# hchautran/SplatFormer

Hardware: AMD Instinct MI355X
Metric: refined renders/sec (100k GS, 800x800) at 1/2/4/8 MI355X; PSNR vs ref (higher is better)
Workload: dtype fp32; 1 GPU; B: 100000 Gaussians SH1, full PTv3 (ptv3_base) + heads, 9 views 800x800, forward; parallelism=scene-dp1, attention=non-flash (K=128, ptv3_base.gin:27)

## Files before the change

### include/sfx.h

```cpp
#ifndef SFX_H_
#define SFX_H_

#include <stddef.h>
#include <stdint.h>

#ifdef __cplusplus
extern "C" {
#endif

#define SFX_OK 0
#define SFX_ERR_INVALID -1
#define SFX_ERR_HIP -2
#define SFX_ERR_WORKSPACE -3

int sfx_abi_version(void);
const char* sfx_last_error(void);

size_t sfx_scan_workspace_bytes(long long n);
long long sfx_lookback_timeouts(void* stream);
int sfx_lookback_release(void* stream);
int sfx_scan_i32(long long n, const int32_t* in, int32_t* out, int inclusive, void* ws, size_t ws_bytes,
                 int32_t* total, void* stream);
int sfx_scan_i64(long long n, const int64_t* in, int64_t* out, int inclusive, void* ws, size_t ws_bytes,
                 int64_t* total, void* stream);
// ... 17 lines not shown
                    const float* v_conic, const float* v_compensation, float* v_mean, float* v_scale,
                    float* v_quat, float* v_cov2d, float* v_cov3d, void* stream);

int sfx_render_prep_project(int n, int num_bases, const float* means, long long ld_means, const float* log_scales,
                            long long ld_scales, const float* quats_raw, long long ld_quats, const float* opac_logit,
                            long long ld_opac, const float* features_dc, long long ld_dc, const float* features_rest,
                            long long ld_rest, const float* camera_to_world, float fx, float fy, float cx,
                            float cy, int img_h, int img_w, int block_width, float* viewmat_out, float* rgbs,
                            float* opacities, float* xys, float* depths, int* radii, float* conics,
                            int* num_tiles_hit, void* stream);

int sfx_isect_emit(int n, const float* xys, const float* depths, const int* radii, const int* cum_tiles_hit,
                   int tiles_x, int tiles_y, int block_width, int64_t* isect_ids, int32_t* gaussian_ids,
                   void* stream);
int sfx_tile_bins(int num_isect, const int64_t* isect_ids_sorted, int num_tiles, int* tile_bins, void* stream);

int sfx_rasterize_fwd(int tiles_x, int tiles_y, int block_width, int img_h, int img_w, const int32_t* gids_sorted,
                      const int* tile_bins, const float* xys, const float* conics, const float* colors,
                      const float* opacity, const float* background, float* final_Ts, int* final_idx,
                      float* out_img, float* out_alpha, void* stream);
int sfx_rasterize_bwd(int tiles_x, int tiles_y, int block_width, int img_h, int img_w, const int32_t* gids_sorted,
                      const int* tile_bins, const float* xys, const float* conics, const float* colors,
                      const float* opacity, const float* background, const float* final_Ts, const int* final_idx,
                      const float* v_out, const float* v_out_alpha, float* v_xy, float* v_xy_abs, float* v_conic,
                      float* v_rgb, float* v_opacity, void* stream);

int sfx_pack_raster_records(int n, const float* xys, const float* conics, const float* colors, const float* opacity,
                            float* records, void* stream);
int sfx_rasterize_fwd_views_packed(int views, int tiles_x, int tiles_y, int block_width, int img_h, int img_w,
                                   const int32_t* gids_sorted, const int* tile_bins, const float* records,
                                   const float* background, int clamp_max1, float* final_Ts, int* final_idx,
                                   float* out_img, float* out_alpha, void* stream);

int sfx_linear(int M, int N, int K, const float* A, long long lda, const int* gather_idx, int num_segments,
               const float* W, long long ldw, const float* bias, const float* scale, const float* shift, int act,
               int act_ncols, const float* R, long long ldr, const int* residual_idx, float* Y, long long ldy,
               float* Ypre, long long ldypre, int groups, long long group_stride_A, long long group_stride_W,
               long long group_stride_bias, long long group_stride_Y, const int* out_row_idx, const float* rowscale,
               int pre_before_act, const unsigned long long* a_amax, unsigned a_tag,
               const unsigned long long* w_amax, unsigned w_tag, unsigned long long* y_amax, unsigned y_tag,
               const float* w_split, const float* w_inv, void* stream);

int sfx_weight_split(int rows, int cols, const float* w, long long ld, float* w_split, float* w_inv, void* stream);

int sfx_amax_f32(int rows, int cols, const float* x, long long ld, unsigned long long* slot, unsigned tag,
                 void* stream);
int sfx_ln_amax_bound(int C, const float* gamma, const float* beta, unsigned long long* slot, unsigned tag,
                      void* stream);

int sfx_gemm_force_config(int cfg, int stream_k);

int sfx_gemm_force_epilogue(int cls);
int sfx_gemm_last_epilogue(void);

int sfx_set_precision(int mode);
int sfx_get_precision(void);

int sfx_linear_bwd_data(int M, int N, int K, const float* dY, long long ldy, const float* Wt, long long ldwt,
                        const float* rowscale, int dact, int dact_ncols, const float* dact_pre, long long ld_pre,
                        float* dX, long long lddx, int accumulate, const float* wt_split, const float* wt_inv,
                        void* stream);
int sfx_linear_wgrad(int M, int N, int K, const float* dY, long long ldy, const float* X, long long ldx, float* dW,
                     long long ldw, float* db, void* stream);
int sfx_linear_wgrad_rs(int M, int N, int K, const float* dY, long long ldy, const float* X, long long ldx,
                        const float* rowscale, float* scaled, float* dW, long long ldw, float* db, void* stream);
int sfx_subm_conv_wgrad(int n, int cin, int cout, const float* dy, long long ldy, const float* x, long long ldx,
                        const int* nbr, const int* pair_in, const int* pair_out, const int* pair_off_host, float* dw,
                        long long ldw, float* db, void* stream);
int sfx_profile_marker(int tag, void* stream);

int sfx_transpose(int rows, int cols, const float* src, long long lds, float* dst, long long ldd, void* stream);
int sfx_subm_conv_bwd_data(int n, int cin, int cout, const float* dy, long long ldy, const int* nbr,
                           const float* weight_t, const int* pair_in, const int* pair_out, const int* pair_off_host,
                           int* centre_ws, float* dx, long long lddx, const float* wt_split, const float* wt_inv,
                           void* stream);
int sfx_window_attention_bwd(int num_windows, int window, int heads, int head_dim, int channels, const float* qkv,
                             const int* order, const int* win, float scale, const float* attn_out, const float* dout,
                             float* dqkv, float* stats, void* stream);
int sfx_window_attention_varlen_bwd(int num_windows, int max_window, int heads, int head_dim, int channels,
                                    const float* qkv, const int* order, const int* win3, float scale,
                                    const float* dout, float* dqkv, float* stats, void* stream);
int sfx_layernorm_bwd(int M, int C, const float* X, long long ldx, const float* gamma, const float* dY,
                      long long ldgy, const float* dR, long long ldr, float eps, float* dX, long long lddx,
                      void* stream);
size_t sfx_layernorm_wgrad_workspace_bytes(int M, int C);
int sfx_layernorm_wgrad(int M, int C, const float* X, long long ldx, const float* dY, long long ldgy, float eps,
                        void* ws, size_t ws_bytes, float* dgamma, float* dbeta, int accumulate, void* stream);
int sfx_cpe_ln_bwd(int M, int C, const float* U, const float* X1, const float* gamma_cpe, const float* gamma1,
                   const float* dX2, const float* dH, float eps, float* dX1, float* dU, void* stream);
size_t sfx_colsum2_workspace_bytes(int M, int C);
int sfx_bn_stats(int M, int C, const float* X, long long ldx, void* ws, size_t ws_bytes, double* sums, void* stream);
int sfx_bn_finalize(int C, double count, const double* sums, const float* gamma, const float* beta, float eps,
                    float momentum, float* running_mean, float* running_var, float* mean_out, float* rstd_out,
                    float* scale_out, float* shift_out, void* stream);
int sfx_affine_act(int M, int C, const float* X, long long ldx, const float* scale, const float* shift, int act,
                   const float* R, long long ldr, const int* ridx, float* Y, long long ldy, void* stream);
int sfx_bn_act_bwd_reduce(int M, int C, const float* X, long long ldx, const float* mean, const float* rstd,
                          const float* gamma, const float* beta, int act, const float* dY, long long ldgy, void* ws,
                          size_t ws_bytes, double* sums, void* stream);
int sfx_bn_act_bwd_apply(int M, int C, const float* X, long long ldx, const float* mean, const float* rstd,
                         const float* gamma, const float* beta, int act, const float* dY, long long ldgy,
                         const double* sums, double count, float* dX, long long lddx, int accumulate, void* stream);
int sfx_segment_max_arg(int m, int C, const int* idx_ptr, const int* sorted_idx, const float* X, float* Y, int* arg,
                        void* stream);
int sfx_segment_max_bwd(int m, int C, const float* dY, const int* arg, float* dX, void* stream);
int sfx_segment_sum(int m, int C, const int* idx_ptr, const int* sorted_idx, const float* X, long long ldx, float* Y,
// ... 211 lines not shown
```

### splatformer_amd/build_lib.py

```python
from __future__ import annotations

import concurrent.futures as cf
import glob
import os
import re
import subprocess
import sys

HERE = os.path.dirname(os.path.abspath(__file__))
CSRC = os.path.join(HERE, "csrc")
ROOT = os.path.dirname(HERE)
BUILD = os.path.join(ROOT, "build", "sfx")
LIB = os.path.join(HERE, "libsfx.so")
ARCH = os.environ.get("SFX_OFFLOAD_ARCH", "gfx950")
HIPCC = os.environ.get("HIPCC", "/opt/rocm/bin/hipcc")

CFLAGS = [
    f"--offload-arch={ARCH}",
    "-O3",
    "-fPIC",
    "-std=c++17",
    "-ffp-contract=fast-honor-pragmas",
    "-munsafe-fp-atomics",
    "-Wno-unused-result",
    f"-I{CSRC}",
    f"-I{os.path.join(ROOT, 'include')}",
]


_INC = re.compile(r'^\s*#\s*include\s*"([^"]+)"', re.M)


def _deps_mtime(path: str, seen=None) -> float:
    seen = set() if seen is None else seen
    if path in seen or not os.path.exists(path):
        return 0.0
    seen.add(path)
    t = os.path.getmtime(path)
    for inc in _INC.findall(open(path, errors="ignore").read()):
        for d in (os.path.dirname(path), CSRC, os.path.join(ROOT, "include")):
            cand = os.path.join(d, inc)
            if os.path.exists(cand):
                t = max(t, _deps_mtime(cand, seen))
                break
    return t


def _flags_stamp() -> float:
    stamp = os.path.join(BUILD, "flags.txt")
    want = " ".join([HIPCC, *CFLAGS])
    have = open(stamp).read() if os.path.exists(stamp) else None
    if have != want:
        with open(stamp, "w") as f:
            f.write(want)
    return os.path.getmtime(stamp)


def _compile(src: str, flags_mtime: float) -> str:
    obj = os.path.join(BUILD, os.path.basename(src).replace(".hip", ".o"))
    if os.path.exists(obj) and os.path.getmtime(obj) >= max(_deps_mtime(src), flags_mtime):
        return obj
    cmd = [HIPCC, *CFLAGS, "-c", src, "-o", obj]
    r = subprocess.run(cmd, capture_output=True, text=True)
    if r.returncode != 0:
        raise RuntimeError(f"hipcc failed for {src}:\n{r.stderr}")
    return obj


def build(verbose: bool = False, jobs: int | None = None) -> str:
    os.makedirs(BUILD, exist_ok=True)
    srcs = sorted(glob.glob(os.path.join(CSRC, "*.hip")))
    hm = _flags_stamp()
    jobs = jobs or min(8, len(srcs))
    with cf.ThreadPoolExecutor(jobs) as ex:
        objs = list(ex.map(lambda s: _compile(s, hm), srcs))
    newest = max(os.path.getmtime(o) for o in objs)
    if not os.path.exists(LIB) or os.path.getmtime(LIB) < newest:
        cmd = [HIPCC, f"--offload-arch={ARCH}", "-shared", "-fPIC", "-o", LIB, *objs]
        r = subprocess.run(cmd, capture_output=True, text=True)
        if r.returncode != 0:
            raise RuntimeError(f"link failed:\n{r.stderr}")
    if verbose:
        print(f"built {LIB}")
    return LIB


if __name__ == "__main__":
    build(verbose=True)
    sys.exit(0)
```

### splatformer_amd/csrc/gemm.hip

```cpp
#include <climits>
#include <cstdlib>
#include <cstring>
#include <type_traits>

#include "gemm_common.h"


namespace {

using namespace sfxg;

inline bool aligned16(const void* p) { return (reinterpret_cast<uintptr_t>(p) & 15) == 0; }

inline bool fits(long long rows, long long ld) { return rows * ld * 4 + 64 < (long long)OOB; }

struct TileCfg {
  int bm, bn, nw;
  float eff;
};
constexpr TileCfg kCfgs[] = {{128, 128, 4, 1.0f}, {128, 96, 4, 0.95f}, {128, 64, 4, 0.8f}, {64, 128, 4, 0.95f},
                             {64, 64, 4, 0.8f},   {256, 128, 8, 1.05f}, {128, 256, 8, 1.05f}};
constexpr int kNumCfgs = sizeof(kCfgs) / sizeof(kCfgs[0]);

thread_local int g_prec = 0;
// ... 204 lines not shown
    for (const TunedLaunch& t : kTuned) {
      if (t.N == a.N && t.K == a.K && 5ll * a.M >= 4ll * t.M && 4ll * a.M <= 5ll * t.M &&
          !((kCfgs[t.cfg].nw == 8) && !split)) {
        a.sk = (t.sk && sk_ok && kCfgs[t.cfg].bm >= 128) ? 1 : 0;
        tiles_m_of(a, kCfgs[t.cfg].bm);
        return t.cfg;
      }
    }
  }
  int best = 0;
  bool best_sk = false;
  double best_cost = 1e300;
  for (int c = 0; c < kNumCfgs; ++c) {
    if (force >= 0 && c != force) continue;
    if (kCfgs[c].nw == 8 && !split) continue;
    const int per_cu = kCfgs[c].nw == 4 ? kPerCu4 : kPerCu8;
    const long long slots = (long long)per_cu * num_cus() / groups;
    const double area = (double)kCfgs[c].bm * kCfgs[c].bn / kCfgs[c].eff * per_cu / 2;
    const long long tiles = (long long)tiles_m_of(a, kCfgs[c].bm) * sfx::ceil_div(a.N, kCfgs[c].bn) * groups;
    const long long rounds = (tiles + slots - 1) / slots;
    double cost = (double)rounds * (nk + 1) * area;
    bool sk = false;
    if (sk_ok && kCfgs[c].bm >= 128) {
      const double sk_cost = ((double)((tiles * nk + slots - 1) / slots) + sk_overhead) * area;
      if (sk_cost < cost || forced_sk == 1) {
        cost = sk_cost;
        sk = true;
      }
    }
    if (cost < best_cost) {
      best_cost = cost;
      best = c;
      best_sk = sk;
    }
  }
  a.sk = best_sk ? 1 : 0;
  tiles_m_of(a, kCfgs[best].bm);
  return best;
}

int forced_epi = -2;
int last_epi = -1;
int pick_epi(const GemmArgs& a, bool vec) {
  if (forced_epi == -2) {
    const char* e = getenv("SFX_GEMM_EPI");
    forced_epi = (e && *e && atoi(e) == 0) ? 0 : -1;
  }
  if (forced_epi == 0 || !vec || a.split != 2 || a.sk) return EPI_GENERAL;
  if (a.pair_mode) return a.pair_store ? EPI_PAIR_STORE : EPI_GENERAL;
  if (a.gidx || a.out_rows || a.ridx || a.Ypre || a.rowscale || a.dact) return EPI_GENERAL;
  return a.act == ACT_NONE ? EPI_LIN : (a.act == ACT_GELU ? EPI_LIN_GELU : EPI_GENERAL);
}

template <int MODE>
void dispatch_mode(GemmArgs a, int groups, bool vec, hipStream_t st) {
  const int cfg = pick_cfg(a, groups, vec);
  a.epi = last_epi = pick_epi(a, vec);
  const bool w8 = kCfgs[cfg].nw == 8;
  switch (MODE) {
    case MODE_DENSE: (w8 ? launch_m0_w8 : launch_m0_w4)(cfg, a, groups, vec, st); break;
    case MODE_GATHER1: (w8 ? launch_m1_w8 : launch_m1_w4)(cfg, a, groups, vec, st); break;
    default: (w8 ? launch_m3_w8 : launch_m3_w4)(cfg, a, groups, vec, st); break;
  }
}

void dispatch(const GemmArgs& a0, int groups, bool vec, hipStream_t st) {
  GemmArgs a = a0;
  static const int dbg = getenv("SFX_GEMM_DEBUG") ? atoi(getenv("SFX_GEMM_DEBUG")) : 0;
  a.dbg = dbg;
  a.split = vec ? split_mode(a.K) : 0;
  if (a.split == 2 && !a.Wsp) a.split = 3;
  if (a.split == 2 && g_prec == 1) a.split = 1;
  last_epi = EPI_GENERAL;
  if (a.pair_mode)
    dispatch_mode<MODE_PAIR>(a, groups, vec, st);
  else if (!a.gidx)
    dispatch_mode<MODE_DENSE>(a, groups, vec, st);
  else if (a.S == 1)
    dispatch_mode<MODE_GATHER1>(a, groups, vec, st);
  else
    launch_m2_w4(3, a, groups, vec, st);
}

__global__ void __launch_bounds__(256) weight_split_kernel(int rows, int cols, const float* __restrict__ src,
                                                           long long ld, float* __restrict__ dst,
                                                           float* __restrict__ inv) {
  const int row = (int)blockIdx.x * 4 + (int)(threadIdx.x >> 6);
  const int lane = threadIdx.x & 63;
  if (row >= rows) return;
  const float* s = src + (long long)row * ld;
  float m = 0.f;
  for (int c = lane * 4; c < cols; c += 256) {
    const float4 v = *reinterpret_cast<const float4*>(s + c);
    m = fmaxf(m, fmaxf(fmaxf(fabsf(v.x), fabsf(v.y)), fmaxf(fabsf(v.z), fabsf(v.w))));
  }
  m = sfx::wave_max(m);
  int e = 0;
  if (m > 0.f && m <= 3.4028235e38f) e = row_exp(m) + 2;
  const float sc = ldexpf(1.f, e);
  uint2* d = reinterpret_cast<uint2*>(dst + (long long)row * cols);
  for (int c = lane * 4; c < cols; c += 256) {
    uint2 t[2];
    split2h(*reinterpret_cast<const float4*>(s + c), sc, t);
    d[c / 2] = t[0];
    d[c / 2 + 1] = t[1];
  }
  if (lane == 0) inv[row] = ldexpf(1.f, -e);
}

constexpr int WG_TILE = 64;

__global__ void __launch_bounds__(THREADS) wgrad_kernel(int M, int N, int K, const float* __restrict__ dY,
                                                        long long ldy, const float* __restrict__ X, long long ldx,
                                                        float* __restrict__ dW, long long ldw, int chunk,
                                                        float* __restrict__ db) {
  __shared__ __attribute__((aligned(16))) float sA[WG_TILE * LDS_STRIDE];
  __shared__ __attribute__((aligned(16))) float sB[WG_TILE * LDS_STRIDE];
  const int tiles_k = (K + WG_TILE - 1) / WG_TILE;
  const int n0 = (blockIdx.x / tiles_k) * WG_TILE, k0 = (blockIdx.x % tiles_k) * WG_TILE;
  const int m_begin = blockIdx.y * chunk;
  const int m_end = min(M, m_begin + chunk);
  const int tid = threadIdx.x, lane = tid & 63, wid = tid >> 6;
// ... 234 lines not shown
                                                            float* __restrict__ out) {
  const long long i = (long long)blockIdx.x * 256 + threadIdx.x;
  if (i >= (long long)M * n4) return;
  const int m = (int)(i / n4), c = (int)(i % n4) * 4;
  const float s = rowscale[m];
  const float4 v = *reinterpret_cast<const float4*>(dY + (long long)m * ldy + c);
  *reinterpret_cast<float4*>(out + i * 4) = make_float4(v.x * s, v.y * s, v.z * s, v.w * s);
}

__global__ void __launch_bounds__(256) transpose_kernel(int rows, int cols, const float* __restrict__ src,
                                                        long long lds, float* __restrict__ dst, long long ldd) {
  __shared__ float t[32][33];
  const int r0 = blockIdx.y * 32, c0 = blockIdx.x * 32;
  const int tx = threadIdx.x & 31, ty = threadIdx.x >> 5;
  for (int i = ty; i < 32; i += 8) {
    const int r = r0 + i, c = c0 + tx;
    t[i][tx] = (r < rows && c < cols) ? src[(long long)r * lds + c] : 0.f;
  }
  __syncthreads();
  for (int i = ty; i < 32; i += 8) {
    const int c = c0 + i, r = r0 + tx;
    if (c < cols && r < rows) dst[(long long)c * ldd + r] = t[tx][i];
  }
}


__global__ void centre_pairs_kernel(int n, const int* __restrict__ nbr, int* __restrict__ gather,
                                    int* __restrict__ scatter) {
  const int i = blockIdx.x * 256 + threadIdx.x;
  if (i >= n) return;
  gather[i] = i;
  scatter[i] = nbr[(long long)i * 27 + 13];
}

}

extern "C" {

int sfx_gemm_force_config(int cfg, int stream_k) {
  SFX_REQUIRE(cfg >= -1 && cfg < kNumCfgs && stream_k >= -1 && stream_k <= 1, "sfx_gemm_force_config: bad values");
  read_force_env();
  forced = cfg;
  forced_sk = stream_k;
  return SFX_OK;
}

int sfx_gemm_force_epilogue(int cls) {
  SFX_REQUIRE(cls == -1 || cls == 0, "sfx_gemm_force_epilogue: class %d (-1 automatic, 0 general)", cls);
  forced_epi = cls;
  return SFX_OK;
}

int sfx_gemm_last_epilogue(void) { return last_epi; }

int sfx_weight_split(int rows, int cols, const float* w, long long ld, float* w_split, float* w_inv, void* stream) {
  SFX_REQUIRE(rows >= 0 && cols > 0 && cols % 4 == 0 && ld >= cols && ld % 4 == 0,
              "sfx_weight_split: bad sizes (cols and ld must be multiples of 4)");
  if (rows == 0) return SFX_OK;
  SFX_REQUIRE(w && w_split && w_inv, "sfx_weight_split: null buffer");
  SFX_REQUIRE((reinterpret_cast<uintptr_t>(w) & 15) == 0 && (reinterpret_cast<uintptr_t>(w_split) & 15) == 0,
              "sfx_weight_split: buffers must be 16-byte aligned");
  weight_split_kernel<<<sfx::ceil_div(rows, 4), 256, 0, sfx::as_stream(stream)>>>(rows, cols, w, ld, w_split, w_inv);
  return sfx::check_launch("sfx_weight_split");
}

int sfx_amax_f32(int rows, int cols, const float* x, long long ld, unsigned long long* slot, unsigned tag,
                 void* stream) {
  SFX_REQUIRE(rows >= 0 && cols >= 0 && ld >= cols, "sfx_amax_f32: bad sizes");
  SFX_REQUIRE(slot && tag != 0, "sfx_amax_f32: null slot or tag 0");
  SFX_REQUIRE(rows == 0 || cols == 0 || x, "sfx_amax_f32: null buffer");
  const AmaxJob j{x, ld, 0, rows, cols, 1, nullptr, 0, 1};
  amax_kernel<<<dim3(amax_blocks(j), 1), 256, 0, sfx::as_stream(stream)>>>(j, j, slot, slot, tag, tag);
  return sfx::check_launch("sfx_amax_f32");
}

int sfx_linear(int M, int N, int K, const float* A, long long lda, const int* gather_idx, int num_segments,
               const float* W, long long ldw, const float* bias, const float* scale, const float* shift, int act,
               int act_ncols, const float* R, long long ldr, const int* residual_idx, float* Y, long long ldy,
               float* Ypre, long long ldypre, int groups, long long group_stride_A, long long group_stride_W,
               long long group_stride_bias, long long group_stride_Y, const int* out_row_idx, const float* rowscale,
               int pre_before_act, const unsigned long long* a_amax, unsigned a_tag,
               const unsigned long long* w_amax, unsigned w_tag, unsigned long long* y_amax, unsigned y_tag,
               const float* w_split, const float* w_inv, void* stream) {
  SFX_REQUIRE(M >= 0 && N > 0 && K > 0, "sfx_linear: bad sizes M=%d N=%d K=%d", M, N, K);
  SFX_REQUIRE(act >= 0 && act <= 3, "sfx_linear: bad activation %d", act);
  SFX_REQUIRE(groups >= 1, "sfx_linear: groups < 1");
  if (M == 0) return SFX_OK;
  SFX_REQUIRE(A && W && Y, "sfx_linear: null buffer");
  const int S = gather_idx ? num_segments : 1;
  SFX_REQUIRE(!gather_idx || (S >= 1 && K % S == 0), "sfx_linear: K must be a multiple of num_segments");
  const int Kseg = K / S;
  SFX_REQUIRE(!gather_idx || Kseg % 4 == 0, "sfx_linear: gathered segment width must be a multiple of 4");
  SFX_REQUIRE(ldw >= K && (gather_idx || lda >= K) && ldy >= N, "sfx_linear: leading dimension too small");
  SFX_REQUIRE(!(scale == nullptr) == !(shift == nullptr), "sfx_linear: scale and shift go together");
  SFX_REQUIRE((gather_idx || fits(M, lda)) && fits(M, ldy) && fits(N, ldw) && (!R || residual_idx || fits(M, ldr)) &&
                  (!Ypre || fits(M, ldypre)),
              "sfx_linear: operand exceeds the 2 GiB buffer-descriptor range");
  GemmArgs a{};
  a.M = M; a.N = N; a.K = K; a.A = A; a.lda = lda; a.gidx = gather_idx; a.S = S; a.Kseg = Kseg; a.gstride = S;
  a.W = W; a.ldw = ldw; a.bias = bias; a.scale = scale; a.shift = shift; a.act = act;
  a.act_ncols = act_ncols < 0 ? N : act_ncols; a.R = R; a.ldr = ldr; a.ridx = residual_idx; a.Y = Y; a.ldy = ldy;
  a.Ypre = Ypre; a.ldypre = ldypre; a.gA = group_stride_A; a.gW = group_stride_W; a.gB = group_stride_bias;
  a.gY = group_stride_Y; a.out_rows = out_row_idx; a.rowscale = rowscale; a.pre_before_act = pre_before_act;
  a.a_amax = a_amax; a.a_tag = a_tag; a.w_amax = w_amax; a.w_tag = w_tag; a.y_amax = y_amax; a.y_tag = y_tag;
  const bool vec = (K % 4 == 0) && (lda % 4 == 0) && (ldw % 4 == 0) && aligned16(A) && aligned16(W) &&
                   (group_stride_A % 4 == 0) && (group_stride_W % 4 == 0);
// ... 272 lines not shown
```

### splatformer_amd/csrc/gemm_common.h

```cpp
#pragma once

#include <type_traits>

#include "common.h"

namespace sfxg {

typedef float floatx16 __attribute__((ext_vector_type(16)));
typedef float floatx4 __attribute__((ext_vector_type(4)));
typedef __bf16 bf16x8 __attribute__((ext_vector_type(8)));

constexpr int BK = 32;
#ifndef SFX_PERCU4
#define SFX_PERCU4 2
#endif
#ifndef SFX_PERCU8
#define SFX_PERCU8 1
#endif
#ifndef SFX_NBUF8
#define SFX_NBUF8 2
#endif
constexpr int kPerCu4 = SFX_PERCU4, kPerCu8 = SFX_PERCU8;
constexpr int LDS_STRIDE = BK + 4;
constexpr int THREADS = 256;
constexpr unsigned OOB = 0x7ffffff0u;
constexpr int RSRC_FLAGS = 0x00020000;

enum Act { ACT_NONE = 0, ACT_GELU = 1, ACT_RELU = 2, ACT_TANH = 3 };
enum Epi { EPI_GENERAL = 0, EPI_LIN = 1, EPI_LIN_GELU = 2, EPI_PAIR_STORE = 3 };

struct GemmArgs {
  int M, N, K;
  const float* A;
  long long lda;
  const int* gidx;
  int S, Kseg, gstride;
  const float* W;
  long long ldw;
  const float* bias;
  const float* scale;
  const float* shift;
  int act, act_ncols;
  const float* R;
  long long ldr;
  const int* ridx;
  float* Y;
  long long ldy;
  float* Ypre;
  long long ldypre;
  long long gA, gW, gB, gY;
  const int* out_rows;
  int pair_mode;
  const int* pair_in;
  const int* pair_out;
  int slice_tile_off[28];
  int slice_pair_off[28];
  int num_slices;
  long long slice_w_stride;
  const float* rowscale;
  int pre_before_act;
  const float* dact_pre;
  long long ld_dact;
  int dact;
  int sk;
  int split;
  const unsigned long long* a_amax;
  const unsigned long long* w_amax;
  unsigned a_tag, w_tag;
  unsigned long long* y_amax;
  unsigned y_tag;
  const float* Wsp;
  long long ldws;
  const float* winv;
  long long gWinv;
  long long slice_winv_stride;
  int tuned, tuned_sk;
  int pair_store;
  int epi;
  int dbg;
};

__device__ __forceinline__ int row_exp(float m) {
  int e = __builtin_amdgcn_frexp_expf(m);
  e = 13 - e;
  return e > 126 ? 126 : (e < -126 ? -126 : e);
}

__device__ __forceinline__ float gelu_erf(float x) {
  const float t = fminf(fabsf(x), 5.65f);
  float q = 2.79405867e-06f;
  q = __builtin_fmaf(q, t, -3.89084234e-05f);
  q = __builtin_fmaf(q, t, 0.000184072458f);
  q = __builtin_fmaf(q, t, 0.000141672252f);
  q = __builtin_fmaf(q, t, -0.00706906663f);
  q = __builtin_fmaf(q, t, 0.0524996631f);
  q = __builtin_fmaf(q, t, 0.459207207f);
  q = __builtin_fmaf(q, t, 1.15110528f);
  const float half_tail = 0.5f * __builtin_amdgcn_exp2f(-(t * q));
  return x >= 0.f ? x * (1.f - half_tail) : (x < -5.65f ? 0.f : x * half_tail);
}
__device__ __forceinline__ float gelu_erf_grad(float x) {
  const float cdf = 0.5f * (1.f + erff(x * 0.70710678118654752f));
  const float pdf = 0.39894228040143268f * expf(-0.5f * x * x);
  return cdf + x * pdf;
}
enum DAct { DACT_NONE = 0, DACT_GELU = 1, DACT_RELU = 2, DACT_TANH_OUT = 3 };
__device__ __forceinline__ float dact_grad(int dact, float pre) {
  if (dact == DACT_GELU) return gelu_erf_grad(pre);
  if (dact == DACT_RELU) return pre > 0.f ? 1.f : 0.f;
  return 1.f - pre * pre;
}

__device__ __forceinline__ __amdgpu_buffer_rsrc_t rsrc(const void* p) {
  const unsigned long long a = reinterpret_cast<unsigned long long>(p);
  const unsigned lo = __builtin_amdgcn_readfirstlane((unsigned)a);
  const unsigned hi = __builtin_amdgcn_readfirstlane((unsigned)(a >> 32));
  void* u = reinterpret_cast<void*>(((unsigned long long)hi << 32) | lo);
  return __builtin_amdgcn_make_buffer_rsrc(u, (short)0, (int)OOB, RSRC_FLAGS);
}

__device__ __forceinline__ __amdgpu_buffer_rsrc_t rsrc_ext(const void* p, unsigned bytes) {
  const unsigned long long a = reinterpret_cast<unsigned long long>(p);
  const unsigned lo = __builtin_amdgcn_readfirstlane((unsigned)a);
  const unsigned hi = __builtin_amdgcn_readfirstlane((unsigned)(a >> 32));
  void* u = reinterpret_cast<void*>(((unsigned long long)hi << 32) | lo);
  return __builtin_amdgcn_make_buffer_rsrc(u, (short)0, (int)__builtin_amdgcn_readfirstlane(bytes), RSRC_FLAGS);
}

__device__ __forceinline__ float4 bload4(__amdgpu_buffer_rsrc_t r, unsigned off) {
  const floatx4 v = __builtin_bit_cast(floatx4, __builtin_amdgcn_raw_buffer_load_b128(r, off, 0, 0));
  return make_float4(v.x, v.y, v.z, v.w);
}
// ... 46 lines not shown
```

### splatformer_amd/csrc/gemm_kernel.h

```cpp
#pragma once
#include <climits>
#include <cstdlib>
#include <cstring>
#include <type_traits>

#include "gemm_common.h"


namespace {

using namespace sfxg;



template <int BM, int BN, int WGM, int NW, bool VEC, int MODE, int SPL, int EPI = EPI_GENERAL>
__global__ void __launch_bounds__(NW * 64, NW == 4 ? 2 : 1) gemm_kernel(GemmArgs p, int tiles_n, int total_tiles) {
  constexpr bool SPLIT = SPL != 0;
  static_assert(EPI == EPI_GENERAL || (SPL == 2 && VEC), "specialised epilogues: fp16x2 operands only");
  static_assert((EPI != EPI_LIN && EPI != EPI_LIN_GELU) || MODE == MODE_DENSE, "EPI_LIN*: dense rows");
  static_assert(EPI != EPI_PAIR_STORE || MODE == MODE_PAIR, "EPI_PAIR_STORE: pair mode");
  constexpr bool F16 = SPL == 2 || SPL == 1;
  constexpr int NTERM = SPL == 1 ? 1 : (F16 ? 2 : 3);
  static_assert(SPL == 0 || SPL == 1 || SPL == 2 || SPL == 3, "operand precision");
  constexpr int NT = NW * 64;
// ... 41 lines not shown
  const unsigned lda32 = (unsigned)p.lda, ldw32 = (unsigned)p.ldw, ldy32 = (unsigned)p.ldy, ldws32 = (unsigned)p.ldws;
  const unsigned ldr32 = (unsigned)p.ldr, ldp32 = (unsigned)p.ldypre;
  const int lrow = tid >> 3, lcol = (tid & 7) * 4;

  struct Tile {
    int m0, n0, M;
    const int* gidx;
    int gstride;
    const int* out_rows;
    const float* W;
    const float* winv;
  };
  auto tile_info = [&](int t) -> Tile {
    Tile ti;
    const int tm = t / tiles_n, tn = t - tm * tiles_n;
    ti.n0 = tn * BN;
    ti.m0 = tm * BM;
    ti.M = p.M;
    ti.gidx = MODE == MODE_DENSE ? nullptr : p.gidx;
    ti.gstride = p.gstride;
    ti.out_rows = p.out_rows;
    ti.W = (F16 ? p.Wsp : p.W) + g * p.gW;
    ti.winv = p.winv ? p.winv + g * p.gWinv : nullptr;
    if constexpr (MODE == MODE_PAIR) {
      int sl = 0;
      for (int q = 1; q < p.num_slices; ++q)
        if (p.slice_tile_off[q] <= tm) sl = q;
      const int base = p.slice_pair_off[sl];
      ti.M = p.slice_pair_off[sl + 1] - base;
      ti.m0 = (tm - p.slice_tile_off[sl]) * BM;
      ti.gidx = p.pair_in + base;
      ti.gstride = 1;
      ti.out_rows = p.pair_out + base;
      ti.W = (F16 ? p.Wsp : p.W) + sl * p.slice_w_stride;
      if (p.winv) ti.winv = p.winv + sl * p.slice_winv_stride;
    }
    return ti;
  };

  int grow[A_ITERS];
  auto load_rows = [&](const Tile& ti, int kt, int (&rows)[A_ITERS]) {
    if constexpr (MODE != MODE_DENSE) {
      const __amdgpu_buffer_rsrc_t rG = rsrc(ti.gidx);
      const int seg = MODE == MODE_GATHERS ? (kt * BK + lcol) / p.Kseg : 0;
#pragma unroll
      for (int i = 0; i < A_ITERS; ++i) {
        const int m = ti.m0 + lrow + RPP * i;
        rows[i] = bload1i(rG, (m < ti.M && seg < p.S) ? ((unsigned)m * (unsigned)ti.gstride + (unsigned)seg) * 4u
                                                      : OOB);
      }
    }
  };

  float4 ra[A_ITERS], rw[W_ITERS];
  auto load_tiles = [&](const Tile& ti, int kt, bool first) {
    const __amdgpu_buffer_rsrc_t rW = rsrc(ti.W);
    const int k = kt * BK + lcol;
    const bool kin = k < K && !(p.dbg & 2);
    int seg = 0, kk = k;
    if constexpr (MODE == MODE_GATHERS) {
      seg = k / p.Kseg;
      kk = k - seg * p.Kseg;
    }
#pragma unroll
    for (int i = 0; i < A_ITERS; ++i) {
      const int m = ti.m0 + lrow + RPP * i;
      const bool mok = m < ti.M;
      unsigned off;
      if constexpr (MODE != MODE_DENSE) {
        const int r = grow[i];
        off = (mok && r >= 0 && kin && seg < p.S) ? ((unsigned)r * lda32 + (unsigned)kk) * 4u : OOB;
      } else {
        off = (mok && kin) ? ((unsigned)m * lda32 + (unsigned)kk) * 4u : OOB;
      }
      if (VEC) {
        ra[i] = bload4(rA, off);
      } else {
        float4 v;
        v.x = bload1(rA, (k + 0 < K) ? off : OOB);
        v.y = bload1(rA, (k + 1 < K) ? off + 4 : OOB);
        v.z = bload1(rA, (k + 2 < K) ? off + 8 : OOB);
        v.w = bload1(rA, (k + 3 < K) ? off + 12 : OOB);
        ra[i] = v;
      }
    }
#pragma unroll
    for (int i = 0; i < W_ITERS; ++i) {
      const int n = ti.n0 + lrow + RPP * i;
      const unsigned off = (n < p.N && kin) ? ((unsigned)n * (F16 ? ldws32 : ldw32) + (unsigned)k) * 4u : OOB;
      if (VEC) {
        rw[i] = bload4(rW, off);
      } else {
        float4 v;
        v.x = bload1(rW, (k + 0 < K) ? off : OOB);
        v.y = bload1(rW, (k + 1 < K) ? off + 4 : OOB);
        v.z = bload1(rW, (k + 2 < K) ? off + 8 : OOB);
        v.w = bload1(rW, (k + 3 < K) ? off + 12 : OOB);
        rw[i] = v;
      }
    }
  };
  int erow[A_ITERS];
  float srow[A_ITERS], thr[A_ITERS];
#pragma unroll
  for (int i = 0; i < A_ITERS; ++i) { erow[i] = INT_MIN; srow[i] = 1.f; thr[i] = 0.f; }
  int sq = 0, cq = 0;
  int sp = 0;
  auto store_tiles = [&](int buf, bool first, int par) {
    if (p.dbg & 8) return;
    if constexpr (SPLIT) {
      const int b = NBUF == 2 ? buf : 0;
      if constexpr (F16) {
        ++sq;
        float m[A_ITERS];
        bool over = false;
#pragma unroll
        for (int i = 0; i < A_ITERS; ++i) {
          m[i] = fmaxf(fmaxf(fabsf(ra[i].x), fabsf(ra[i].y)), fmaxf(fabsf(ra[i].z), fabsf(ra[i].w)));
          over |= m[i] > thr[i];
        }
        bool dec = false;
        if (first || __builtin_amdgcn_ballot_w64(over) != 0) {
#pragma unroll
          for (int i = 0; i < A_ITERS; ++i) {
            float mr = m[i];
            mr = fmaxf(mr, __int_as_float(__builtin_amdgcn_mov_dpp(__float_as_int(mr), 0xB1, 0xF, 0xF, false)));
            mr = fmaxf(mr, __int_as_float(__builtin_amdgcn_mov_dpp(__float_as_int(mr), 0x4E, 0xF, 0xF, false)));
            mr = fmaxf(mr, __int_as_float(__builtin_amdgcn_mov_dpp(__float_as_int(mr), 0x141, 0xF, 0xF, false)));
            int e = first ? INT_MIN : erow[i];
            float fac = 1.f;
            bool chg = first;
            if (mr > 0.f && mr <= 3.4028235e38f) {
              int e2 = 13 - __builtin_amdgcn_frexp_expf(mr);
              e2 = e2 > 126 ? 126 : (e2 < -126 ? -126 : e2);
              if (e == INT_MIN) {
                e = e2;
                chg = true;
              } else if (mr * srow[i] > 65504.f) {
                fac = ldexpf(1.f, e2 - e);
                e = e2;
                chg = true;
                dec = true;
              }
            }
            erow[i] = e;
            const bool set = e != INT_MIN;
            srow[i] = set ? ldexpf(1.f, e) : 1.f;
            thr[i] = set ? ldexpf(65504.f, -e) : 0.f;
            if ((tid & 7) == 0) {
              s_fac[b * BM + lrow + RPP * i] = fac;
              if (chg) s_inv[par * BM + lrow + RPP * i] = set ? ldexpf(1.f, -e) : 1.f;
            }
          }
        } else if ((tid & 7) == 0) {
#pragma unroll
          for (int i = 0; i < A_ITERS; ++i) s_fac[b * BM + lrow + RPP * i] = 1.f;
        }
        if (__builtin_amdgcn_ballot_w64(dec) != 0 && lane == 0) s_flag[b] = sq;
#pragma unroll
        for (int i = 0; i < A_ITERS; ++i) {
          uint2 t[2];
          split2h(ra[i], srow[i], t);
// ... 214 lines not shown
      const unsigned br = n < p.N ? (mb * ldr32 + (unsigned)n) * 4u : OOBX;
#pragma unroll
      for (int r = 0; r < 16; ++r) rv[r] = bload1(rRd, br + rowc(r) * ldr32 * 4u);
    };
    float rv[2][16];
    load_r(0, rv[0]);
#pragma unroll
    for (int blk = 0; blk < MB * NB; ++blk) {
      const int a = blk / NB, b = blk % NB;
      if (blk + 1 < MB * NB) load_r(blk + 1, rv[(blk + 1) & 1]);
      const bool do_act = ti.n0 + wn * WN + b * 32 + l32 < p.act_ncols;
      const float c1 = p.scale ? escale[b] : 1.f;
      const float c0 = ebias[b] * c1 + eshift[b];
#pragma unroll
      for (int r = 0; r < 16; ++r) {
        float v = __builtin_fmaf(acc[a][b][r], c1, c0);
        if constexpr (EPI == EPI_LIN_GELU) v = do_act ? gelu_erf(v) : v;
        v = has_r ? v + rv[blk & 1][r] : v;
        ymax = fmaxf(ymax, fabsf(v));
        acc[a][b][r] = v;
      }
    }
    __builtin_amdgcn_sched_barrier(0);
#pragma unroll
    for (int a = 0; a < MB; ++a) {
      const unsigned mb = (unsigned)(ti.m0 + wm * WM + a * 32 + 4 * h);
#pragma unroll
      for (int b = 0; b < NB; ++b) {
        const int n = ti.n0 + wn * WN + b * 32 + l32;
        const unsigned by = n < p.N ? (mb * ldy32 + (unsigned)n) * 4u : OOBX;
#pragma unroll
        for (int r = 0; r < 16; ++r) bstore1(rYd, by + rowc(r) * ldy32 * 4u, acc[a][b][r]);
      }
    }
  };

  auto pair_store_epilogue = [&](const Tile& ti) {
    const unsigned pbase = (unsigned)(ti.out_rows - p.pair_out);
    const __amdgpu_buffer_rsrc_t rYd = rsrc_ext(Y, (pbase + (unsigned)ti.M) * ldy32 * 4u);
#pragma unroll
    for (int a = 0; a < MB; ++a) {
      const unsigned mb = pbase + (unsigned)(ti.m0 + wm * WM + a * 32 + 4 * h);
#pragma unroll
      for (int b = 0; b < NB; ++b) {
        const int n = ti.n0 + wn * WN + b * 32 + l32;
        const unsigned by = n < p.N ? (mb * ldy32 + (unsigned)n) * 4u : OOBX;
#pragma unroll
        for (int r = 0; r < 16; ++r) bstore1(rYd, by + rowc(r) * ldy32 * 4u, acc[a][b][r]);
      }
    }
  };

  auto epilogue = [&](const Tile& ti, bool partial, bool owner0) {
    if (p.dbg & 4) return;
    unscale();
    if constexpr (EPI == EPI_LIN || EPI == EPI_LIN_GELU) {
      lin_epilogue(ti);
      return;
    }
    if constexpr (EPI == EPI_PAIR_STORE) {
      pair_store_epilogue(ti);
      return;
    }
    if constexpr (MODE != MODE_PAIR) {
      if (!ti.out_rows) {
        direct_epilogue(ti, partial, owner0);
        return;
      }
    }
    if constexpr (MODE == MODE_PAIR) {
      const __amdgpu_buffer_rsrc_t rO = rsrc(ti.out_rows);
      const int pbase = (int)(ti.out_rows - p.pair_out);
#pragma unroll
      for (int a = 0; a < MB; ++a) {
        int orow[16];
        bool ok[16];
#pragma unroll
        for (int r = 0; r < 16; ++r) {
          const int mt = ti.m0 + wm * WM + a * 32 + (r & 3) + 8 * (r >> 2) + 4 * h;
          ok[r] = mt < ti.M;
          orow[r] = p.pair_store ? pbase + mt : bload1i(rO, ok[r] ? (unsigned)mt * 4u : OOB);
        }
#pragma unroll
        for (int b = 0; b < NB; ++b) {
          const int n = ti.n0 + wn * WN + b * 32 + l32;
          const bool nok = n < p.N;
          if (p.pair_store) {
#pragma unroll
            for (int r = 0; r < 16; ++r)
              bstore1(rY, (nok && ok[r]) ? ((unsigned)orow[r] * ldy32 + (unsigned)n) * 4u : OOB, acc[a][b][r]);
            continue;
          }
#pragma unroll
          for (int r = 0; r < 16; ++r)
            __builtin_amdgcn_raw_ptr_buffer_atomic_fadd_f32(
                acc[a][b][r], rY, (nok && ok[r]) ? ((unsigned)orow[r] * ldy32 + (unsigned)n) * 4u : OOB, 0, 0);
        }
      }
      return;
    }
    resolve_rows(ti);
#pragma unroll
    for (int a = 0; a < MB; ++a) {
#pragma unroll
      for (int b = 0; b < NB; ++b) {
        const int n = ti.n0 + wn * WN + b * 32 + l32;
        const bool nok = n < p.N;
// ... 85 lines not shown
          for (int r = 0; r < 16; ++r) {
            const int m = mrow[a][r];
            bstore1(rY, (nok && m >= 0) ? ((unsigned)m * ldy32 + (unsigned)n) * 4u : OOB, v[r]);
          }
        }
      }
    }
  };

  auto compute_split = [&](int buf, int s0, int s1) {
    const int bb = NBUF == 2 ? buf : 0;
    typedef __attribute__((ext_vector_type(8))) _Float16 f16x8;
    typedef typename std::conditional<F16, f16x8, bf16x8>::type frag_t;
#pragma unroll
    for (int s = s0; s < s1; ++s) {
      frag_t af[MB][NTERM], wf[NB][NTERM];
#pragma unroll
      for (int q = 0; q < NTERM; ++q) {
#pragma unroll
        for (int a = 0; a < MB; ++a) {
          const int r = wm * WM + a * 32 + l32;
          af[a][q] = __builtin_bit_cast(
              frag_t, *reinterpret_cast<const uint4*>(sAs + ((bb * NTERM + q) * BM) * 64 + swz(r, 4 * s + 2 * h)));
        }
#pragma unroll
        for (int b = 0; b < NB; ++b) {
          const int r = wn * WN + b * 32 + l32;
          wf[b][q] = __builtin_bit_cast(
              frag_t, *reinterpret_cast<const uint4*>(sWs + ((bb * NTERM + q) * BN) * 64 + swz(r, 4 * s + 2 * h)));
        }
      }
      if constexpr (F16) {
        constexpr int QA[3] = {1, 0, 0}, QW[3] = {0, 1, 0};
#pragma unroll
        for (int j = SPL == 1 ? 2 : 0; j < 3; ++j)
#pragma unroll
          for (int a = 0; a < MB; ++a)
#pragma unroll
            for (int b = 0; b < NB; ++b)
              acc[a][b] = __builtin_amdgcn_mfma_f32_32x32x16_f16(af[a][QA[j]], wf[b][QW[j]], acc[a][b], 0, 0, 0);
      } else {
        constexpr int QA[6] = {2, 1, 0, 1, 0, 0}, QW[6] = {0, 1, 2, 0, 1, 0};
#pragma unroll
        for (int j = 0; j < 6; ++j)
#pragma unroll
          for (int a = 0; a < MB; ++a)
#pragma unroll
            for (int b = 0; b < NB; ++b)
              acc[a][b] = __builtin_amdgcn_mfma_f32_32x32x16_bf16(af[a][QA[j]], wf[b][QW[j]], acc[a][b], 0, 0, 0);
      }
    }
  };
  auto compute = [&](int buf) {
    if (p.dbg & 1) return;
    if constexpr (F16) {
      ++cq;
      const int b = NBUF == 2 ? buf : 0;
      if (__builtin_amdgcn_readfirstlane(s_flag[b]) == cq) {
#pragma unroll
        for (int a = 0; a < MB; ++a)
#pragma unroll
          for (int gq = 0; gq < 4; ++gq) {
            const float4 f = *reinterpret_cast<const float4*>(s_fac + b * BM + wm * WM + a * 32 + 8 * gq + 4 * h);
#pragma unroll
            for (int bb = 0; bb < NB; ++bb) {
              acc[a][bb][4 * gq + 0] *= f.x;
              acc[a][bb][4 * gq + 1] *= f.y;
              acc[a][bb][4 * gq + 2] *= f.z;
              acc[a][bb][4 * gq + 3] *= f.w;
            }
          }
      }
    }
    if constexpr (SPLIT) {
      compute_split(buf, 0, BK / 16);
      return;
    }
    const float* a_lds = &sA[buf][(wm * WM + l32) * LDS_STRIDE + h * 16];
    const float* w_lds = &sW[buf][(wn * WN + l32) * LDS_STRIDE + h * 16];
#pragma unroll
    for (int c = 0; c < 4; ++c) {
      float4 af[MB], wf[NB];
#pragma unroll
      for (int a = 0; a < MB; ++a) af[a] = *reinterpret_cast<const float4*>(a_lds + a * 32 * LDS_STRIDE + 4 * c);
#pragma unroll
      for (int b = 0; b < NB; ++b) wf[b] = *reinterpret_cast<const float4*>(w_lds + b * 32 * LDS_STRIDE + 4 * c);
#pragma unroll
      for (int a = 0; a < MB; ++a)
#pragma unroll
        for (int b = 0; b < NB; ++b) {
          acc[a][b] = __builtin_amdgcn_mfma_f32_32x32x2f32(af[a].x, wf[b].x, acc[a][b], 0, 0, 0);
          acc[a][b] = __builtin_amdgcn_mfma_f32_32x32x2f32(af[a].y, wf[b].y, acc[a][b], 0, 0, 0);
          acc[a][b] = __builtin_amdgcn_mfma_f32_32x32x2f32(af[a].z, wf[b].z, acc[a][b], 0, 0, 0);
          acc[a][b] = __builtin_amdgcn_mfma_f32_32x32x2f32(af[a].w, wf[b].w, acc[a][b], 0, 0, 0);
        }
    }
  };

  const int nwg = (int)gridDim.x;
  const int lid = (nwg % 8 == 0) ? (int)(blockIdx.x % 8) * (nwg / 8) + (int)(blockIdx.x / 8) : (int)blockIdx.x;
  int t, kb = 0, ke = nk;
  long long it_end = 0;
  if (p.sk) {
    const long long total_it = (long long)total_tiles * nk;
    const long long it0 = total_it * lid / nwg;
    it_end = total_it * (lid + 1) / nwg;
    if (it0 >= it_end) return;
    t = (int)(it0 / nk);
    kb = (int)(it0 - (long long)t * nk);
    ke = (int)min((long long)nk, kb + (it_end - it0));
  } else {
    t = lid;
    if (t >= total_tiles) return;
  }
  constexpr bool per_tile_rows = MODE == MODE_GATHER1 || MODE == MODE_PAIR;
  Tile ti = tile_info(t);
  load_rows(ti, kb, grow);
  load_tiles(ti, kb, true);
  store_tiles(0, true, sp);
  __syncthreads();
  int buf = 0;
  while (true) {
    int nt, nke = nk;
    bool has_next;
    if (p.sk) {
      nt = t + 1;
      has_next = (long long)nt * nk < it_end;
      if (has_next) nke = (int)min((long long)nk, it_end - (long long)nt * nk);
    } else {
      nt = t + nwg;
      has_next = nt < total_tiles;
    }
    const Tile tn = has_next ? tile_info(nt) : ti;
    int grow_next[A_ITERS];
    if constexpr (per_tile_rows) load_rows(tn, 0, grow_next);
    zero_acc();
    for (int kt = kb; kt + 1 < ke; ++kt) {
      if constexpr (MODE == MODE_GATHERS) load_rows(ti, kt + 1, grow);
      load_tiles(ti, kt + 1, false);
      __builtin_amdgcn_sched_barrier(0);
      compute(buf);
      __builtin_amdgcn_sched_barrier(0);
      if constexpr (NBUF == 1) __syncthreads();
      store_tiles(buf ^ 1, false, sp);
      __syncthreads();
      if constexpr (NBUF == 2) buf ^= 1;
    }
    pre_epilogue(ti);
    if (has_next) {
      if constexpr (per_tile_rows) {
#pragma unroll
        for (int i = 0; i < A_ITERS; ++i) grow[i] = grow_next[i];
      } else {
        load_rows(tn, 0, grow);
      }
      load_tiles(tn, 0, true);
    }
    __builtin_amdgcn_sched_barrier(0);
    compute(buf);
    __builtin_amdgcn_sched_barrier(0);
    epilogue(ti, kb != 0 || ke != nk, kb == 0);
    if (!has_next) break;
    if constexpr (NBUF == 1) __syncthreads();
    __builtin_amdgcn_sched_barrier(0);
    store_tiles(buf ^ 1, true, sp ^ 1);
    __syncthreads();
    if constexpr (NBUF == 2) buf ^= 1;
    sp ^= 1;
    t = nt;
    ti = tn;
    kb = 0;
    ke = nke;
  }
  if (p.y_amax) {
    __shared__ float ywaves[NW];
    sfx::publish_amax(ymax, p.y_amax, p.y_tag, ywaves);
  }
}
template <int BM, int BN, int WGM, int NW, int MODE>
void launch_f16x2(const GemmArgs& a, dim3 grid, int tiles_n, int total, hipStream_t st) {
  constexpr int T = NW * 64;
  if constexpr (MODE == MODE_DENSE) {
    if (a.epi == EPI_LIN) {
      gemm_kernel<BM, BN, WGM, NW, true, MODE, 2, EPI_LIN><<<grid, T, 0, st>>>(a, tiles_n, total);
      return;
    }
    if (a.epi == EPI_LIN_GELU) {
      gemm_kernel<BM, BN, WGM, NW, true, MODE, 2, EPI_LIN_GELU><<<grid, T, 0, st>>>(a, tiles_n, total);
      return;
    }
  }
  if constexpr (MODE == MODE_PAIR) {
    if (a.epi == EPI_PAIR_STORE) {
      gemm_kernel<BM, BN, WGM, NW, true, MODE, 2, EPI_PAIR_STORE><<<grid, T, 0, st>>>(a, tiles_n, total);
      return;
    }
  }
  gemm_kernel<BM, BN, WGM, NW, true, MODE, 2><<<grid, T, 0, st>>>(a, tiles_n, total);
}

template <int BM, int BN, int WGM, int NW, int MODE>
void launch(GemmArgs a, int groups, bool vec, hipStream_t st) {
  const bool split = a.split != 0;
  const int tiles_m = tiles_m_of(a, BM);
  const int tiles_n = (int)sfx::ceil_div(a.N, BN);
  const int total = tiles_m * tiles_n;
  const int per_cu = NW == 4 ? kPerCu4 : kPerCu8;
  const int slots = per_cu * num_cus() / groups > 0 ? per_cu * num_cus() / groups : 1;
  int grid_x;
  if (a.sk) {
    const long long iters = (long long)total * sfx::ceil_div(a.K, BK);
    grid_x = (int)(iters < slots ? iters : slots);
    if (grid_x >= 8) grid_x = grid_x / 8 * 8;
    if (grid_x < 1) grid_x = 1;
    if (!a.pair_mode)
      (void)hipMemset2DAsync(a.Y, (size_t)a.ldy * 4, 0, (size_t)a.N * 4, (size_t)a.M, st);
  } else {
    const int per = (total + slots - 1) / slots;
    grid_x = total > 0 ? (total + per - 1) / per : 1;
    if (grid_x >= 8) grid_x = (grid_x + 7) / 8 * 8;
  }
  dim3 grid(grid_x, 1, groups);
  if constexpr (NW == 8) {
    if (a.split == 2)
      launch_f16x2<BM, BN, WGM, 8, MODE>(a, grid, tiles_n, total, st);
    else if (a.split == 1)
      gemm_kernel<BM, BN, WGM, 8, true, MODE, 1><<<grid, 512, 0, st>>>(a, tiles_n, total);
    else
      gemm_kernel<BM, BN, WGM, 8, true, MODE, 3><<<grid, 512, 0, st>>>(a, tiles_n, total);
  } else {
    if (vec && a.split == 2)
      launch_f16x2<BM, BN, WGM, 4, MODE>(a, grid, tiles_n, total, st);
    else if (vec && a.split == 1)
      gemm_kernel<BM, BN, WGM, 4, true, MODE, 1><<<grid, 256, 0, st>>>(a, tiles_n, total);
    else if (vec && split)
      gemm_kernel<BM, BN, WGM, 4, true, MODE, 3><<<grid, 256, 0, st>>>(a, tiles_n, total);
    else if (vec)
      gemm_kernel<BM, BN, WGM, 4, true, MODE, 0><<<grid, 256, 0, st>>>(a, tiles_n, total);
    else
      gemm_kernel<BM, BN, WGM, 4, false, MODE, 0><<<grid, 256, 0, st>>>(a, tiles_n, total);
  }
}

}
```

### splatformer_amd/ptv3_ops.py

```python
from __future__ import annotations

import contextlib
import ctypes
import os
from typing import List, Optional, Sequence, Tuple

import numpy as np
import torch
from torch import Tensor

from . import _lib
from ._lib import call, ptr, stream

ACT_NONE, ACT_GELU, ACT_RELU, ACT_TANH = 0, 1, 2, 3
GEMM_NUM_CONFIGS = 7


def gemm_force_config(cfg: int = -1, stream_k: int = -1) -> None:
    call("sfx_gemm_force_config", cfg, stream_k)


def gemm_force_epilogue(cls: int = -1) -> None:
    call("sfx_gemm_force_epilogue", cls)


EPI_GENERAL, EPI_LIN, EPI_LIN_GELU, EPI_PAIR_STORE = 0, 1, 2, 3


def gemm_last_epilogue() -> int:
    return int(_lib.fn("sfx_gemm_last_epilogue")())


PRECISIONS = {"fp32": 0, "amp": 1}


def get_precision() -> str:
    m = _lib.fn("sfx_get_precision")()
    return {v: k for k, v in PRECISIONS.items()}[m]


@contextlib.contextmanager
def precision(mode: str):
    if mode not in PRECISIONS:
        raise ValueError(f"precision {mode!r}: expected one of {sorted(PRECISIONS)}")
    prev = _lib.fn("sfx_get_precision")()
    call("sfx_set_precision", PRECISIONS[mode])
    try:
        yield
    finally:
        call("sfx_set_precision", prev)
ORDER_TYPES = {"z": 0, "z-trans": 1, "hilbert": 2, "hilbert-trans": 3}


AMAX_SUB = 64
_AMAX_RING = 4096
_amax_state: dict = {}


def new_amax(device) -> Tuple[int, int]:
    st = _amax_state.get(device)
    if st is None:
        buf = torch.zeros(_AMAX_RING * AMAX_SUB, dtype=torch.int64, device=device)
        st = _amax_state[device] = [buf, 0, 0]
    buf = st[0]
    st[1] = (st[1] + 1) % _AMAX_RING
    st[2] = st[2] + 1 if st[2] < 0x7FFFFFFF else 1
    return buf.data_ptr() + 8 * AMAX_SUB * st[1], st[2]


def _own_slot(device) -> Tuple[Tensor, Tuple[int, int]]:
    buf = torch.zeros(AMAX_SUB, dtype=torch.int64, device=device)
    return buf, (buf.data_ptr(), 1)


def weight_amax(w: Tensor) -> Tuple[int, int]:
    key = (w.data_ptr(), w._version, tuple(w.shape))
# ... 843 lines not shown
```

Measured before the change: 689.7 renders/s.

## Prefetch second K-tile of next persistent GEMM tile and compile out debug switches

For the 128x256, 8-wave, double-buffered f16x2-split GEMM with a fast epilogue, the kernel now loads the first two K-slices of the next tile before running the epilogue. The second slice is stored to shared memory right after the first compute of the new tile, so the global-load latency at tile boundaries is hidden behind the epilogue. The debug/ablation branches (SFX_GEMM_DEBUG bits) are now compiled out by default, which removes runtime checks from the hot loops. A separate ablate build variant and a forced grid cap are added for experiments. The extra prefetch registers raise register pressure and could reduce occupancy.

```diff
diff --git a/include/sfx.h b/include/sfx.h
--- a/include/sfx.h
+++ b/include/sfx.h
@@ -93,6 +93,10 @@
 
 int sfx_gemm_force_epilogue(int cls);
 int sfx_gemm_last_epilogue(void);
+
+int sfx_gemm_force_grid(int workgroups);
+
+int sfx_gemm_ablation_built(void);
 
 int sfx_set_precision(int mode);
 int sfx_get_precision(void);
diff --git a/splatformer_amd/build_lib.py b/splatformer_amd/build_lib.py
--- a/splatformer_amd/build_lib.py
+++ b/splatformer_amd/build_lib.py
@@ -56,11 +56,11 @@
     return os.path.getmtime(stamp)
 
 
-def _compile(src: str, flags_mtime: float) -> str:
-    obj = os.path.join(BUILD, os.path.basename(src).replace(".hip", ".o"))
+def _compile(src: str, flags_mtime: float, out_dir: str = BUILD, extra: tuple = ()) -> str:
+    obj = os.path.join(out_dir, os.path.basename(src).replace(".hip", ".o"))
     if os.path.exists(obj) and os.path.getmtime(obj) >= max(_deps_mtime(src), flags_mtime):
         return obj
-    cmd = [HIPCC, *CFLAGS, "-c", src, "-o", obj]
+    cmd = [HIPCC, *CFLAGS, *extra, "-c", src, "-o", obj]
     r = subprocess.run(cmd, capture_output=True, text=True)
     if r.returncode != 0:
         raise RuntimeError(f"hipcc failed for {src}:\n{r.stderr}")
@@ -85,6 +85,41 @@
     return LIB
 
 
+def build_variant(name: str, extra_flags, patterns=("gemm", "gemm_k*"), verbose: bool = False) -> str:
+    import fnmatch
+    build()
+    out_dir = os.path.join(ROOT, "build", f"exp_{name}")
+    os.makedirs(out_dir, exist_ok=True)
+    hm = os.path.getmtime(os.path.join(BUILD, "flags.txt"))
+    stamp = os.path.join(out_dir, "flags.txt")
+    want = " ".join(extra_flags)
+    if not os.path.exists(stamp) or open(stamp).read() != want:
+        with open(stamp, "w") as f:
+            f.write(want)
+    hm = max(hm, os.path.getmtime(stamp))
+    srcs = sorted(glob.glob(os.path.join(CSRC, "*.hip")))
+    base = lambda s: os.path.basename(s)[:-len(".hip")]
+    own = [s for s in srcs if any(fnmatch.fnmatch(base(s), p) for p in patterns)]
+    with cf.ThreadPoolExecutor(min(8, len(own) or 1)) as ex:
+        objs = list(ex.map(lambda s: _compile(s, hm, out_dir, tuple(extra_flags)), own))
+    objs += [os.path.join(BUILD, base(s) + ".o") for s in srcs if s not in own]
+    lib = os.path.join(HERE, f"exp_{name}.so")
+    r = subprocess.run([HIPCC, f"--offload-arch={ARCH}", "-shared", "-fPIC", "-o", lib, *objs],
+                       capture_output=True, text=True)
+    if r.returncode != 0:
+        raise RuntimeError(f"link failed:\n{r.stderr}")
+    if verbose:
+        print(f"built {lib}")
+    return lib
+
+
+def build_ablate(verbose: bool = False) -> str:
+    return build_variant("ablate", ["-DSFX_GEMM_ABLATE=1"], verbose=verbose)
+
+
 if __name__ == "__main__":
-    build(verbose=True)
+    if "--ablate" in sys.argv[1:]:
+        build_ablate(verbose=True)
+    else:
+        build(verbose=True)
     sys.exit(0)
diff --git a/splatformer_amd/csrc/gemm.hip b/splatformer_amd/csrc/gemm.hip
--- a/splatformer_amd/csrc/gemm.hip
+++ b/splatformer_amd/csrc/gemm.hip
@@ -280,6 +280,19 @@
   return a.act == ACT_NONE ? EPI_LIN : (a.act == ACT_GELU ? EPI_LIN_GELU : EPI_GENERAL);
 }
 
+int forced_grid = -1;
+
+int ablation_bits() {
+  const char* e = getenv("SFX_GEMM_DEBUG");
+  const int bits = (e && *e) ? atoi(e) : 0;
+  if (bits != 0 && !SFX_GEMM_ABLATE) {
+    fprintf(stderr, "libsfx: SFX_GEMM_DEBUG=%d ignored: this library is built without the GEMM timing-ablation "
+                    "switches (build the ablate variant, python -m splatformer_amd.build_lib --ablate)\n", bits);
+    return 0;
+  }
+  return bits;
+}
+
 template <int MODE>
 void dispatch_mode(GemmArgs a, int groups, bool vec, hipStream_t st) {
   const int cfg = pick_cfg(a, groups, vec);
@@ -294,8 +307,9 @@
 
 void dispatch(const GemmArgs& a0, int groups, bool vec, hipStream_t st) {
   GemmArgs a = a0;
-  static const int dbg = getenv("SFX_GEMM_DEBUG") ? atoi(getenv("SFX_GEMM_DEBUG")) : 0;
+  static const int dbg = ablation_bits();
   a.dbg = dbg;
+  a.grid_cap = forced_grid > 0 ? forced_grid : 0;
   a.split = vec ? split_mode(a.K) : 0;
   if (a.split == 2 && !a.Wsp) a.split = 3;
   if (a.split == 2 && g_prec == 1) a.split = 1;
@@ -636,6 +650,15 @@
 }
 
 int sfx_gemm_last_epilogue(void) { return last_epi; }
+
+int sfx_gemm_force_grid(int workgroups) {
+  SFX_REQUIRE(workgroups == -1 || workgroups >= 1, "sfx_gemm_force_grid: %d workgroups (-1 default, or >= 1)",
+              workgroups);
+  forced_grid = workgroups;
+  return SFX_OK;
+}
+
+int sfx_gemm_ablation_built(void) { return SFX_GEMM_ABLATE ? 1 : 0; }
 
 int sfx_weight_split(int rows, int cols, const float* w, long long ld, float* w_split, float* w_inv, void* stream) {
   SFX_REQUIRE(rows >= 0 && cols > 0 && cols % 4 == 0 && ld >= cols && ld % 4 == 0,
diff --git a/splatformer_amd/csrc/gemm_common.h b/splatformer_amd/csrc/gemm_common.h
--- a/splatformer_amd/csrc/gemm_common.h
+++ b/splatformer_amd/csrc/gemm_common.h
@@ -21,6 +21,13 @@
 #define SFX_NBUF8 2
 #endif
 constexpr int kPerCu4 = SFX_PERCU4, kPerCu8 = SFX_PERCU8;
+#ifndef SFX_GEMM_ABLATE
+#define SFX_GEMM_ABLATE 0
+#endif
+#define SFX_GEMM_DBG(bit) (SFX_GEMM_ABLATE != 0 && (p.dbg & (bit)) != 0)
+#ifndef SFX_GEMM_PF2
+#define SFX_GEMM_PF2 1
+#endif
 constexpr int LDS_STRIDE = BK + 4;
 constexpr int THREADS = 256;
 constexpr unsigned OOB = 0x7ffffff0u;
@@ -78,6 +85,7 @@
   int pair_store;
   int epi;
   int dbg;
+  int grid_cap;
 };
 
 __device__ __forceinline__ int row_exp(float m) {
diff --git a/splatformer_amd/csrc/gemm_kernel.h b/splatformer_amd/csrc/gemm_kernel.h
--- a/splatformer_amd/csrc/gemm_kernel.h
+++ b/splatformer_amd/csrc/gemm_kernel.h
@@ -117,11 +117,14 @@
     }
   };
 
+  constexpr bool PF2 = SFX_GEMM_PF2 != 0 && NW == 8 && NBUF == 2 && BM == 128 && BN == 256 && SPL == 2 &&
+                       EPI != EPI_GENERAL;
   float4 ra[A_ITERS], rw[W_ITERS];
-  auto load_tiles = [&](const Tile& ti, int kt, bool first) {
+  float4 ra2[PF2 ? A_ITERS : 1], rw2[PF2 ? W_ITERS : 1];
+  auto load_tiles = [&](const Tile& ti, int kt, bool first, auto& ra, auto& rw) {
     const __amdgpu_buffer_rsrc_t rW = rsrc(ti.W);
     const int k = kt * BK + lcol;
-    const bool kin = k < K && !(p.dbg & 2);
+    const bool kin = k < K && !SFX_GEMM_DBG(2);
     int seg = 0, kk = k;
     if constexpr (MODE == MODE_GATHERS) {
       seg = k / p.Kseg;
@@ -171,8 +174,8 @@
   for (int i = 0; i < A_ITERS; ++i) { erow[i] = INT_MIN; srow[i] = 1.f; thr[i] = 0.f; }
   int sq = 0, cq = 0;
   int sp = 0;
-  auto store_tiles = [&](int buf, bool first, int par) {
-    if (p.dbg & 8) return;
+  auto store_tiles = [&](int buf, bool first, int par, const auto& ra, const auto& rw) {
+    if (SFX_GEMM_DBG(8)) return;
     if constexpr (SPLIT) {
       const int b = NBUF == 2 ? buf : 0;
       if constexpr (F16) {
@@ -493,7 +496,7 @@
   };
 
   auto epilogue = [&](const Tile& ti, bool partial, bool owner0) {
-    if (p.dbg & 4) return;
+    if (SFX_GEMM_DBG(4)) return;
     unscale();
     if constexpr (EPI == EPI_LIN || EPI == EPI_LIN_GELU) {
       lin_epilogue(ti);
@@ -685,7 +688,7 @@
     }
   };
   auto compute = [&](int buf) {
-    if (p.dbg & 1) return;
+    if (SFX_GEMM_DBG(1)) return;
     if constexpr (F16) {
       ++cq;
       const int b = NBUF == 2 ? buf : 0;
@@ -749,10 +752,11 @@
   constexpr bool per_tile_rows = MODE == MODE_GATHER1 || MODE == MODE_PAIR;
   Tile ti = tile_info(t);
   load_rows(ti, kb, grow);
-  load_tiles(ti, kb, true);
-  store_tiles(0, true, sp);
+  load_tiles(ti, kb, true, ra, rw);
+  store_tiles(0, true, sp, ra, rw);
   __syncthreads();
   int buf = 0;
+  bool pre1 = false;
   while (true) {
     int nt, nke = nk;
     bool has_next;
@@ -768,14 +772,26 @@
     int grow_next[A_ITERS];
     if constexpr (per_tile_rows) load_rows(tn, 0, grow_next);
     zero_acc();
-    for (int kt = kb; kt + 1 < ke; ++kt) {
+    int kt = kb;
+    if constexpr (PF2) {
+      if (pre1 && kt + 1 < ke) {
+        __builtin_amdgcn_sched_barrier(0);
+        compute(buf);
+        __builtin_amdgcn_sched_barrier(0);
+        store_tiles(buf ^ 1, false, sp, ra2, rw2);
+        __syncthreads();
+        buf ^= 1;
+        ++kt;
+      }
+    }
+    for (; kt + 1 < ke; ++kt) {
       if constexpr (MODE == MODE_GATHERS) load_rows(ti, kt + 1, grow);
-      load_tiles(ti, kt + 1, false);
+      load_tiles(ti, kt + 1, false, ra, rw);
       __builtin_amdgcn_sched_barrier(0);
       compute(buf);
       __builtin_amdgcn_sched_barrier(0);
       if constexpr (NBUF == 1) __syncthreads();
-      store_tiles(buf ^ 1, false, sp);
+      store_tiles(buf ^ 1, false, sp, ra, rw);
       __syncthreads();
       if constexpr (NBUF == 2) buf ^= 1;
     }
@@ -787,7 +803,8 @@
       } else {
         load_rows(tn, 0, grow);
       }
-      load_tiles(tn, 0, true);
+      load_tiles(tn, 0, true, ra, rw);
+      if constexpr (PF2) load_tiles(tn, 1, false, ra2, rw2);
     }
     __builtin_amdgcn_sched_barrier(0);
     compute(buf);
@@ -796,10 +813,11 @@
     if (!has_next) break;
     if constexpr (NBUF == 1) __syncthreads();
     __builtin_amdgcn_sched_barrier(0);
-    store_tiles(buf ^ 1, true, sp ^ 1);
+    store_tiles(buf ^ 1, true, sp ^ 1, ra, rw);
     __syncthreads();
     if constexpr (NBUF == 2) buf ^= 1;
     sp ^= 1;
+    pre1 = true;
     t = nt;
     ti = tn;
     kb = 0;
@@ -853,6 +871,7 @@
     grid_x = total > 0 ? (total + per - 1) / per : 1;
     if (grid_x >= 8) grid_x = (grid_x + 7) / 8 * 8;
   }
+  if (a.grid_cap > 0 && grid_x > a.grid_cap) grid_x = a.grid_cap;
   dim3 grid(grid_x, 1, groups);
   if constexpr (NW == 8) {
     if (a.split == 2)
diff --git a/splatformer_amd/ptv3_ops.py b/splatformer_amd/ptv3_ops.py
--- a/splatformer_amd/ptv3_ops.py
+++ b/splatformer_amd/ptv3_ops.py
@@ -22,6 +22,14 @@
 
 def gemm_force_epilogue(cls: int = -1) -> None:
     call("sfx_gemm_force_epilogue", cls)
+
+
+def gemm_force_grid(workgroups: int = -1) -> None:
+    call("sfx_gemm_force_grid", workgroups)
+
+
+def gemm_ablation_built() -> bool:
+    return bool(_lib.fn("sfx_gemm_ablation_built")())
 
 
 EPI_GENERAL, EPI_LIN, EPI_LIN_GELU, EPI_PAIR_STORE = 0, 1, 2, 3
```

Result: no change. 693.1 renders/s, median of 6 (+0.5%).
